# zhaozijie2022/LocoTouch

Measured on AMD Instinct MI355X. Metric: env-steps/sec (whole node), TransportTeacher 4096 envs/GPU, higher is better.
Workload: dtype f32

## Files before the change

locotouch_amd/_abi.py:

```python
from __future__ import annotations

import ctypes
import os
import re

_HERE = os.path.dirname(os.path.abspath(__file__))
REPO = os.path.dirname(_HERE)
LIB_PATH = os.environ.get("LOCOTOUCH_AMD_LIB", os.path.join(_HERE, "_lib", "liblocotouch_env.so"))

_SCALARS = {"int": ctypes.c_int, "int32_t": ctypes.c_int32, "int64_t": ctypes.c_int64, "uint8_t": ctypes.c_uint8,
            "uint32_t": ctypes.c_uint32, "uint64_t": ctypes.c_uint64, "size_t": ctypes.c_size_t, "float": ctypes.c_float,
            "double": ctypes.c_double}
_DECL = re.compile(r"(?:const\s+)?(\w+)\s*((?:\*\s*(?:const\b\s*)?)*)(\w*)\s*((?:\[[^\]]*\]\s*)*)")


def _ctype(decl, structs, opaque, consts, typed, param):
    m = _DECL.fullmatch(decl.strip())
    if not m:
        return None
    base, stars, name, dims = m.groups()
    depth = stars.count("*")
    try:
        dims = [sum(int(t) if t.strip().isdigit() else consts[t.strip()] for t in d.split("+")) for d in re.findall(r"\[([^\]]*)\]", dims)]
    except KeyError:
# ... 42 lines not shown
    protos = {}
    for stmt in filter(None, (x.strip() for x in rest.split(";"))):
        m = re.fullmatch(r"(.*?)\b(\w+)\s*\(([^()]*)\)", stmt, flags=re.S)
        if not m:
            if stmt == "}":
                continue
            raise ImportError(f"cannot parse declaration {stmt!r}")
        ret, name, args = m.groups()
        res = (None, None) if ret.strip() == "void" else _ctype(ret, structs, opaque, consts, typed, param=False)
        args = [] if args.strip() == "void" else [_ctype(a, structs, opaque, consts, typed, param=True) for a in args.split(",")]
        if res is None or None in args:
            raise ImportError(f"cannot type prototype {name}: {' '.join(stmt.split())!r}")
        protos[name] = (res[1], [t for _, t in args])
    return consts, structs, protos


class _CfgMethods(ctypes.Structure):
    def copy(self) -> "LtCfg":
        new = LtCfg()
        ctypes.memmove(ctypes.byref(new), ctypes.byref(self), ctypes.sizeof(self))
        for attr in ("extra_reward_terms", "extra_termination_terms", "extra_observation_terms", "reward_term_params"):
            if hasattr(self, attr):
                v = getattr(self, attr)
                setattr(new, attr, dict(v) if isinstance(v, dict) else list(v))
        return new

    def to_dict(self) -> dict:
        def py(v):
            return [py(x) for x in v] if hasattr(v, "__len__") else v

        return {name: py(getattr(self, name)) for name, *_ in self._fields_ if not name.startswith("_")}


_ENV_VALUE_QUERIES = (
    "lt_abi_version", "lt_cfg_sizeof", "lt_cfg_num_presets", "lt_cfg_preset_id", "lt_cfg_obs_dim", "lt_cfg_tactile_dim", "lt_last_error",
    "lt_wgrad_splits", "lt_wgrad_ws_floats", "lt_elu_backward_bias_ws_floats", "lt_head_wgrad_ws_floats", "lt_adam_clip_step_ws_floats",
    "lt_elu_backward_bias_nblk", "lt_head_wgrad_nblk", "lt_mlp_backward_blocks", "lt_env_kernel_name", "lt_mlp_kernel_name")

HEADERS = (
    ("", "lt_env.h", False, _ENV_VALUE_QUERIES, ("lt_cfg", "lt_view", "lt_mlp_desc", "lt_render_view", "lt_render_desc")),
    ("OBS_NORM", "lt_obs_norm.h", False, (), ()),
    ("STUDENT", "lt_student.h", True, ("lt_student_step_launches",), ("lt_student_desc", "lt_student_params")),
    ("COLLECT", "lt_collect.h", False, (), ()),
    ("LEDGER", "lt_ledger.h", False, (), ()),
    ("CNN_TRAIN", "lt_cnn_train.h", False, ("lt_cnn_launches",), ("lt_cnn_desc", "lt_cnn_params", "lt_cnn_grads")),
    ("BC", "lt_bc.h", False, (), ()),
    ("LSTM", "lt_lstm.h", False, (), ()),
    ("MEMORY", "lt_memory.h", False, (), ("lt_memory_net",)),
    ("MEMORY_SEQ", "lt_memory_seq.h", False, ("lt_memory_seq_backward_units",), ("lt_memory_seq_net", "lt_memory_seq_grad")),
    ("MEMORY_GRU", "lt_memory_gru.h", False, ("lt_memory_gru_seq_backward_units",),
     ("lt_memory_gru_net", "lt_memory_gru_seq_net", "lt_memory_gru_seq_grad")),
    ("POLICY", "lt_policy.h", True, ("lt_policy_step_launches",), ("lt_policy_desc", "lt_policy_memory")),
    ("PPO_OPTS", "lt_ppo_opts.h", False, (), ()),
)


def _bind(table, include_dir):
    bound, seen, env_structs = [], set(), None
    for prefix, fname, uses_env_structs, queries, _ in table:
        path, queries = os.path.join(include_dir, fname), frozenset(queries)
        consts, structs, sigs = parse_header(open(path).read(), structs=env_structs if uses_env_structs else None, bases={"lt_cfg": _CfgMethods})
        if not prefix:
            env_structs = structs
        for name in sorted(queries - set(sigs)):
            raise ImportError(f"include/{fname}: the value query {name} named in _abi.HEADERS is not declared there")
        for name, (restype, _) in sigs.items():
            if name in seen:
                raise ImportError(f"include/{fname}: {name} repeats an entry point of an earlier header")
            if restype is not ctypes.c_int and (prefix or name not in queries):
                raise ImportError(f"include/{fname}: {name} returns no int (a new value query of lt_env.h belongs in _abi.HEADERS)")
        seen.update(sigs)
        bound.append((path, consts, structs, sigs, queries))
    return bound


ALL_SIGNATURES: dict = {}
ALL_VALUE_QUERIES: set = set()
for (_prefix, _, _, _, _published), (_path, _consts, _structs, _sigs, _queries) in zip(HEADERS, _bind(HEADERS, os.path.join(REPO, "include"))):
    _p = _prefix + "_" if _prefix else ""
    globals().update(_consts)
    globals().update({_p + "HEADER": _path, _p + "CONSTS": _consts, _p + "SIGNATURES": _sigs, _p + "VALUE_QUERIES": _queries})
    globals().update({_structs[_c].__name__: _structs[_c] for _c in _published})
    if not _prefix:
        STRUCTS, EXPORTS = _structs, list(_sigs)
    ALL_SIGNATURES.update(_sigs)
    ALL_VALUE_QUERIES |= _queries

_lib = None
_calls: dict = {}


def load() -> ctypes.CDLL:
    global _lib
    if _lib is not None:
        return _lib
    if not os.path.exists(LIB_PATH):
        raise ImportError(f"{LIB_PATH} is missing: run `python -c 'import __graft_entry__ as g; g.build()'` "
                          "(the HIP extension is mandatory, there is no CPU fallback)")
    lib = ctypes.CDLL(LIB_PATH)
    for name, (restype, argtypes) in ALL_SIGNATURES.items():
        fn = getattr(lib, name)
        fn.restype, fn.argtypes = restype, argtypes
        if name not in ALL_VALUE_QUERIES:
            _calls[name] = (fn, [ptr if t is ctypes.c_void_p else _ref if issubclass(t, ctypes._Pointer) and issubclass(t._type_, ctypes.Structure)
                                 else None for t in argtypes])
    if lib.lt_cfg_sizeof() != ctypes.sizeof(LtCfg):
# ... 77 lines not shown
```

locotouch_amd/csrc/lt_ppo.hip:

```cpp
#include <hip/hip_runtime.h>
#include <math.h>
#include <stdint.h>

#include "lt_env.h"
#include "lt_host_check.h"
#include "lt_internal.h"

namespace {

constexpr int MAX_A = 16;
constexpr float kHalfLog2Pi = 0.91893853320467274178f;

__device__ __forceinline__ float lt_sigma_of_log(float log_std) { return (float)exp((double)log_std); }

template <bool LOG, bool NORM>
__global__ __launch_bounds__(256) void lt_ppo_loss_kernel(const float* __restrict__ mu, const float* __restrict__ stdp, const float* __restrict__ value,
                                                          const float* __restrict__ actions, const float* __restrict__ old_logp,
                                                          const float* __restrict__ adv, const float* __restrict__ returns,
                                                          const float* __restrict__ old_values, const float* __restrict__ old_mu,
                                                          const float* __restrict__ old_sigma, const long long* __restrict__ idx,
                                                          long long M, int A, float clip, float vcoef, int clipped_value,
                                                          const float* __restrict__ adv_stats, float* __restrict__ dmu, float* __restrict__ dvalue, float* __restrict__ acc) {
  const long long row = (long long)blockIdx.x * 256 + threadIdx.x;
  const bool ok = row < M;
  const long long src = (ok && idx) ? idx[row] : row;
  __shared__ float sigma_lds[MAX_A];
  if constexpr (LOG) {
    if ((int)threadIdx.x < A) sigma_lds[threadIdx.x] = lt_sigma_of_log(stdp[threadIdx.x]);
    __syncthreads();
  }
  float part[4 + MAX_A];
  float amax_mu = 0.f, amax_v = 0.f;
#pragma unroll
  for (int i = 0; i < 4 + MAX_A; ++i) part[i] = 0.f;
  if (ok) {
    const float inv_m = 1.f / (float)M;
    float logp = 0.f, kl = 0.f;
    float z[MAX_A], isg[MAX_A];
#pragma unroll
    for (int a = 0; a < MAX_A; ++a) {
      if (a < A) {
        const float sg = LOG ? sigma_lds[a] : stdp[a], m = mu[row * A + a], x = actions[src * A + a];
        const float om = old_mu[src * A + a], os = old_sigma[src * A + a];
        isg[a] = 1.f / sg;
        z[a] = (x - m) * isg[a];
        if constexpr (LOG) logp += -0.5f * z[a] * z[a] - stdp[a] - kHalfLog2Pi;
        else logp += -0.5f * z[a] * z[a] - __logf(sg) - kHalfLog2Pi;
        {
#pragma clang fp reciprocal(off)
          kl += logf(sg / os + 1.0e-5f) + (os * os + (om - m) * (om - m)) / (2.f * sg * sg) - 0.5f;
        }
      }
    }
    float advr = adv[src];
    if constexpr (NORM) advr = (advr - adv_stats[0]) * adv_stats[1];
    const float ratio = __expf(logp - old_logp[src]);
    const float s1 = -advr * ratio;
    const float rc = fminf(fmaxf(ratio, 1.f - clip), 1.f + clip);
    const float s2 = -advr * rc;
    const bool inside = ratio >= 1.f - clip && ratio <= 1.f + clip;
    const float dsurr_dratio = (s1 > s2 || inside) ? -advr : 0.f;
    const float dlogp = dsurr_dratio * ratio * inv_m;
#pragma unroll
    for (int a = 0; a < MAX_A; ++a) {
      if (a < A) {
        dmu[row * A + a] = dlogp * z[a] * isg[a];
        amax_mu = fmaxf(amax_mu, fabsf(dlogp * z[a] * isg[a]));
        if constexpr (LOG) part[4 + a] = dlogp * (z[a] * z[a] - 1.f);
        else part[4 + a] = dlogp * (z[a] * z[a] - 1.f) * isg[a];
      }
    }
    const float v = value[row], R = returns[src];
    float vl, dv;
    if (clipped_value) {
      const float ov = old_values[src];
      const float dcl = fminf(fmaxf(v - ov, -clip), clip);
      const float vc = ov + dcl;
      const float l1 = (v - R) * (v - R), l2 = (vc - R) * (vc - R);
      const bool in_v = (v - ov) >= -clip && (v - ov) <= clip;
      vl = fmaxf(l1, l2);
      dv = (l1 > l2 || in_v) ? 2.f * (v - R) : 0.f;
    } else {
      vl = (R - v) * (R - v);
      dv = 2.f * (v - R);
    }
    dvalue[row] = vcoef * dv * inv_m;
    amax_v = fabsf(vcoef * dv * inv_m);
    part[0] = fmaxf(s1, s2);
    part[1] = vl;
    part[2] = kl;
  }
  __shared__ float red[4][4 + MAX_A];
  const int lane = threadIdx.x & 63, wave = threadIdx.x >> 6;
#pragma unroll
  for (int i = 0; i < 4 + MAX_A; ++i) {
    float v = part[i];
#pragma unroll
    for (int off = 32; off > 0; off >>= 1) v += __shfl_xor(v, off, 64);
    if (lane == 0) red[wave][i] = v;
  }
#pragma unroll
  for (int off = 32; off > 0; off >>= 1) {
    amax_mu = fmaxf(amax_mu, __shfl_xor(amax_mu, off, 64));
    amax_v = fmaxf(amax_v, __shfl_xor(amax_v, off, 64));
  }
  __shared__ float redm[4][2];
  if (lane == 0) { redm[wave][0] = amax_mu; redm[wave][1] = amax_v; }
  __syncthreads();
  if (threadIdx.x < 4 + A && threadIdx.x != 3) {
    const int i = threadIdx.x;
    atomicAdd(acc + i, red[0][i] + red[1][i] + red[2][i] + red[3][i]);
  } else if (threadIdx.x >= 64 && threadIdx.x < 66) {
    const int j = threadIdx.x - 64;
    atomicMax((unsigned*)acc + 20 + j, __float_as_uint(fmaxf(fmaxf(redm[0][j], redm[1][j]), fmaxf(redm[2][j], redm[3][j]))));
  }
}

__global__ __launch_bounds__(64) void lt_ppo_finalize_kernel(const float* __restrict__ acc, const float* __restrict__ stdp, int A, float inv_m,
                                                             float vcoef, float ecoef, int std_is_log, float* __restrict__ out) {
  const int a = threadIdx.x;
  float e = 0.f;
  if (a < A && std_is_log) {
    e = 0.5f + kHalfLog2Pi + stdp[a];
    out[8 + a] = acc[4 + a] - ecoef;
  } else if (a < A) {
    const float sg = stdp[a];
    e = 0.5f + kHalfLog2Pi + logf(sg);
    out[8 + a] = acc[4 + a] - ecoef / sg;
  }
  for (int off = 32; off > 0; off >>= 1) e += __shfl_xor(e, off, 64);
  if (a == 0) {
    const float surr = acc[0] * inv_m, vl = acc[1] * inv_m;
    out[0] = surr + vcoef * vl - ecoef * e;
    out[1] = surr; out[2] = vl; out[3] = e; out[4] = acc[2] * inv_m;
  }
}

constexpr int EB_ROWS = 48;

__global__ __launch_bounds__(256) void lt_elu_bwd_bias_kernel(const float* da, const float* __restrict__ a, long long M, int N, float alpha,
                                                              float* dz, float* __restrict__ ws, float* __restrict__ amax) {
  const int n4 = N >> 2, lanes = 256 / n4;
  const int c4 = threadIdx.x % n4, rl = threadIdx.x / n4;
  const long long r0 = (long long)blockIdx.x * EB_ROWS;
  float4 sum = {0.f, 0.f, 0.f, 0.f};
  float mx = 0.f;
  if (rl < lanes) {
    for (int r = rl; r < EB_ROWS; r += lanes) {
      const long long row = r0 + r;
      if (row >= M) break;
      const float4 g = ((const float4*)(da + row * N))[c4], y = ((const float4*)(a + row * N))[c4];
      float4 o;
      o.x = g.x * (y.x > 0.f ? 1.f : y.x + alpha);
      o.y = g.y * (y.y > 0.f ? 1.f : y.y + alpha);
      o.z = g.z * (y.z > 0.f ? 1.f : y.z + alpha);
      o.w = g.w * (y.w > 0.f ? 1.f : y.w + alpha);
      ((float4*)(dz + row * N))[c4] = o;
      sum.x += o.x; sum.y += o.y; sum.z += o.z; sum.w += o.w;
      mx = fmaxf(fmaxf(mx, fmaxf(fabsf(o.x), fabsf(o.y))), fmaxf(fabsf(o.z), fabsf(o.w)));
    }
  }
  __shared__ float4 red[256];
  __shared__ float redm[4];
  red[threadIdx.x] = sum;
  if (amax) {
#pragma unroll
    for (int off = 32; off > 0; off >>= 1) mx = fmaxf(mx, __shfl_xor(mx, off, 64));
    if ((threadIdx.x & 63) == 0) redm[threadIdx.x >> 6] = mx;
  }
  __syncthreads();
  if (amax && threadIdx.x == 0) amax[blockIdx.x] = fmaxf(fmaxf(redm[0], redm[1]), fmaxf(redm[2], redm[3]));
  if (threadIdx.x < n4) {
    float4 t = red[threadIdx.x];
    for (int l = 1; l < lanes; ++l) {
      const float4 u = red[l * n4 + threadIdx.x];
      t.x += u.x; t.y += u.y; t.z += u.z; t.w += u.w;
    }
    ((float4*)(ws + (long long)blockIdx.x * N))[threadIdx.x] = t;
  }
}

constexpr int SUM_MAX_JOBS = 24;
struct SumJobs {
  const float* ws[SUM_MAX_JOBS];
  float* out0[SUM_MAX_JOBS];
  float* out1[SUM_MAX_JOBS];
  long long stride[SUM_MAX_JOBS];
  int nblk[SUM_MAX_JOBS], count[SUM_MAX_JOBS], split[SUM_MAX_JOBS], first[SUM_MAX_JOBS + 1];
// ... 186 lines not shown
    }
  }
  __syncthreads();
  const float coef = s_coef;
  const long long base = (long long)blockIdx.x * AD_PER_BLOCK;
  for (int k = threadIdx.x; k < AD_PER_BLOCK; k += 256) {
    const long long i = base + k;
    if (i >= n) break;
    float gi = g[i] * coef;
    g[i] = gi;
    const float pi = p[i];
    if (wd != 0.f) gi += wd * pi;
    const float mi = m[i] + (1.f - b1) * (gi - m[i]);
    const float vi = b2 * v[i] + (1.f - b2) * gi * gi;
    m[i] = mi;
    v[i] = vi;
    p[i] = pi - step_size * (mi / (sqrtf(vi) / bc2_sqrt + eps));
  }
}

__global__ __launch_bounds__(64) void lt_std_from_log_kernel(const float* __restrict__ log_std, int A, float* __restrict__ stdp) {
  if ((int)threadIdx.x < A) stdp[threadIdx.x] = lt_sigma_of_log(log_std[threadIdx.x]);
}

__device__ __forceinline__ double lt_block_sum_f64(double v, double* red) {
#pragma unroll
  for (int off = 32; off > 0; off >>= 1) v += __shfl_xor(v, off, 64);
  __syncthreads();
  if ((threadIdx.x & 63) == 0) red[threadIdx.x >> 6] = v;
  __syncthreads();
  return (red[0] + red[1]) + (red[2] + red[3]);
}

__global__ __launch_bounds__(256) void lt_adv_stats_kernel(const float* __restrict__ adv, const long long* __restrict__ idx, long long M,
                                                           float* __restrict__ stats) {
#pragma clang fp reciprocal(off)
  __shared__ double red[4];
  const long long base = (long long)blockIdx.x * M;
  double s = 0.0;
  for (long long r = threadIdx.x; r < M; r += 256) s += (double)adv[idx ? idx[base + r] : base + r];
  const double mean = lt_block_sum_f64(s, red) / (double)M;
  double q = 0.0;
  for (long long r = threadIdx.x; r < M; r += 256) {
    const double d = (double)adv[idx ? idx[base + r] : base + r] - mean;
    q += d * d;
  }
  const double var = lt_block_sum_f64(q, red) / (double)(M - 1);
  if (threadIdx.x == 0) {
    stats[2 * blockIdx.x] = (float)mean;
    stats[2 * blockIdx.x + 1] = (float)(1.0 / (sqrt(var) + (double)1.0e-8f));
  }
}

__global__ __launch_bounds__(64) void lt_ppo_lr_rule_kernel(const float* __restrict__ kl_mean, float desired, float lr_min, float lr_max, float factor,
                                                            float* __restrict__ lr, float* __restrict__ stats, const float* __restrict__ scalars,
                                                            float* __restrict__ dstd_out, int A) {
  if (dstd_out && scalars && (int)threadIdx.x < A) dstd_out[threadIdx.x] = scalars[8 + threadIdx.x];
  if (threadIdx.x != 0) return;
  if (kl_mean && desired > 0.f) {
#pragma clang fp reciprocal(off)
    const float kl = *kl_mean;
    float v = *lr;
    if (kl > desired * 2.f) v = fmaxf(lr_min, v / factor);
    else if (kl < desired * 0.5f && kl > 0.f) v = fminf(lr_max, v * factor);
    *lr = v;
  }
  if (stats && scalars) { stats[0] += scalars[2]; stats[1] += scalars[1]; stats[2] += scalars[3]; }
}

}

extern "C" int lt_ppo_lr_rule(const float* kl_mean, float desired_kl, float lr_min, float lr_max, float factor, float* lr, float* stats,
                              const float* scalars, float* dstd_out, int num_actions, void* stream) {
  if (!lr || factor <= 1.f || num_actions < 0 || num_actions > MAX_A) return einval("lt_ppo_lr_rule: invalid argument");
  hipLaunchKernelGGL(lt_ppo_lr_rule_kernel, dim3(1), dim3(64), 0, (hipStream_t)stream, kl_mean, desired_kl, lr_min, lr_max, factor, lr, stats, scalars,
                     dstd_out, num_actions);
  return launch_status();
}

static int elu_backward_bias(const float* da, const float* a, int64_t M, int N, float alpha, float* dz, float* db, float* ws, float* amax, void* stream);
extern "C" int lt_elu_backward_bias(const float* da, const float* a, int64_t M, int N, float alpha, float* dz, float* db, float* ws, void* stream) {
  return elu_backward_bias(da, a, M, N, alpha, dz, db, ws, nullptr, stream);
}
extern "C" int lt_elu_backward_bias2(const float* da, const float* a, int64_t M, int N, float alpha, float* dz, float* db, float* ws, float* amax_blocks,
                                     void* stream) {
  return elu_backward_bias(da, a, M, N, alpha, dz, db, ws, amax_blocks, stream);
}
static int elu_backward_bias(const float* da, const float* a, int64_t M, int N, float alpha, float* dz, float* db, float* ws, float* amax, void* stream) {
  if (!da || !a || !dz || !ws || M < 1 || N < 4 || (N & 3) || N > 1024)
    return einval("lt_elu_backward_bias: invalid argument (N a multiple of 4, 4 <= N <= 1024)");
  const int nblk = (int)((M + EB_ROWS - 1) / EB_ROWS);
  hipLaunchKernelGGL(lt_elu_bwd_bias_kernel, dim3((unsigned)nblk), dim3(256), 0, (hipStream_t)stream, da, a, (long long)M, N, alpha, dz, ws, amax);
  if (db) launch_one_sum(ws, nblk, (long long)N, N, N, db, nullptr, (hipStream_t)stream);
  return launch_status();
}

extern "C" int64_t lt_head_wgrad_ws_floats(int64_t M, int n, int k) { return ((M + HW_ROWS - 1) / HW_ROWS) * ((int64_t)n * k + HW_MAX_N); }

extern "C" int lt_head_wgrad(const float* dy, const float* x, int x_split, int64_t M, int n, int k, float* dw, float* db, float* ws, void* stream) {
  if (!dy || !x || !ws || M < 1 || n < 1 || n > HW_MAX_N || k < 4 || (k & 3) || k > 1024)
    return einval("lt_head_wgrad: invalid argument (1 <= n <= 16, k a multiple of 4, 4 <= k <= 1024)");
  const int nblk = (int)((M + HW_ROWS - 1) / HW_ROWS), k4 = k / 4, lanes = 256 / k4;
  const int nn = n <= 1 ? 1 : (n <= 4 ? 4 : (n <= 8 ? 8 : (n <= 12 ? 12 : 16)));
  const size_t lds = (size_t)lanes * nn * k4 * 16 + (size_t)lanes * nn * 4;
  if (const int e = lt_ensure_dynamic_lds((const void*)lt_head_wgrad_kernel<16>, 72 * 1024)) {
    lt_set_error(hipGetErrorString((hipError_t)e));
    return LT_EHIP;
  }
  if (lds > 72 * 1024) return einval("lt_head_wgrad: n * k too large for one block's LDS partials");
  const dim3 g((unsigned)nblk), b(256);
  hipStream_t st = (hipStream_t)stream;
  switch (nn) {
    case 1: hipLaunchKernelGGL(lt_head_wgrad_kernel<1>, g, b, lds, st, dy, x, x_split, (long long)M, n, k, ws); break;
    case 4: hipLaunchKernelGGL(lt_head_wgrad_kernel<4>, g, b, lds, st, dy, x, x_split, (long long)M, n, k, ws); break;
    case 8: hipLaunchKernelGGL(lt_head_wgrad_kernel<8>, g, b, lds, st, dy, x, x_split, (long long)M, n, k, ws); break;
    case 12: hipLaunchKernelGGL(lt_head_wgrad_kernel<12>, g, b, lds, st, dy, x, x_split, (long long)M, n, k, ws); break;
    default: hipLaunchKernelGGL(lt_head_wgrad_kernel<16>, g, b, lds, st, dy, x, x_split, (long long)M, n, k, ws); break;
  }
  if (dw) launch_one_sum(ws, nblk, (long long)n * k + HW_MAX_N, n * k + n, n * k, dw, db, st);
  return launch_status();
// ... 60 lines not shown

static int ppo_loss(const float* mu, const float* stdp, const float* value, const float* actions, const float* old_logp,
                    const float* adv, const float* returns, const float* old_values, const float* old_mu, const float* old_sigma,
                    const int64_t* idx, int64_t M, int A, float clip, float value_loss_coef, float entropy_coef, int use_clipped_value_loss,
                    int std_is_log, const float* adv_stats, float* dmu, float* dvalue, float* acc, float* out, void* stream) {
  const hipError_t e = hipMemsetAsync(acc, 0, sizeof(float) * (4 + MAX_A + 4), (hipStream_t)stream);
  if (e != hipSuccess) { lt_set_error(hipGetErrorString(e)); return LT_EHIP; }
  const dim3 grid((unsigned)((M + 255) / 256));
#define LT_PPO_LOSS_LAUNCH(LOG, NORM)                                                                                                      \
  hipLaunchKernelGGL((lt_ppo_loss_kernel<LOG, NORM>), grid, dim3(256), 0, (hipStream_t)stream, mu, stdp, value, actions, old_logp, adv, returns, \
                     old_values, old_mu, old_sigma, (const long long*)idx, (long long)M, A, clip, value_loss_coef, use_clipped_value_loss,   \
                     adv_stats, dmu, dvalue, acc)
  if (std_is_log && adv_stats) LT_PPO_LOSS_LAUNCH(true, true);
  else if (std_is_log) LT_PPO_LOSS_LAUNCH(true, false);
  else if (adv_stats) LT_PPO_LOSS_LAUNCH(false, true);
  else LT_PPO_LOSS_LAUNCH(false, false);
#undef LT_PPO_LOSS_LAUNCH
  if (out)
    hipLaunchKernelGGL(lt_ppo_finalize_kernel, dim3(1), dim3(64), 0, (hipStream_t)stream, acc, stdp, A, 1.f / (float)M, value_loss_coef, entropy_coef,
                       std_is_log ? 1 : 0, out);
  return launch_status();
}

extern "C" int lt_ppo_loss(const float* mu, const float* stdp, const float* value, const float* actions, const float* old_logp, const float* adv,
                           const float* returns, const float* old_values, const float* old_mu, const float* old_sigma, const int64_t* idx,
                           int64_t M, int A, float clip, float value_loss_coef, float entropy_coef, int use_clipped_value_loss, float* dmu, float* dvalue,
                           float* acc, float* out, void* stream) {
  if (!mu || !stdp || !value || !actions || !old_logp || !adv || !returns || !old_values || !old_mu || !old_sigma || !dmu || !dvalue || !acc ||
      M < 1 || A < 1 || A > MAX_A)
    return einval("lt_ppo_loss: invalid argument (1 <= num_actions <= 16)");
  return ppo_loss(mu, stdp, value, actions, old_logp, adv, returns, old_values, old_mu, old_sigma, idx, M, A, clip, value_loss_coef,
                  entropy_coef, use_clipped_value_loss, 0, nullptr, dmu, dvalue, acc, out, stream);
}

extern "C" int lt_ppo_loss_opts(const float* mu, const float* stdp, const float* value, const float* actions, const float* old_logp,
                                const float* adv, const float* returns, const float* old_values, const float* old_mu, const float* old_sigma,
                                const int64_t* idx, int64_t M, int A, float clip, float value_loss_coef, float entropy_coef,
                                int use_clipped_value_loss, int std_is_log, const float* adv_stats, float* dmu, float* dvalue, float* acc,
                                float* out, void* stream) {
  const char* fn = "lt_ppo_loss_opts";
  const ptr_check ptrs[] = {{"mu", mu, 4}, {"std", stdp, 4}, {"value", value, 4}, {"actions", actions, 4}, {"old_logp", old_logp, 4}, {"adv", adv, 4},
                            {"returns", returns, 4}, {"old_values", old_values, 4}, {"old_mu", old_mu, 4}, {"old_sigma", old_sigma, 4},
                            {"dmu", dmu, 4}, {"dvalue", dvalue, 4}, {"acc", acc, 4}};
  if (const int rc = check_ptrs(fn, "", ptrs)) return rc;
  if ((uintptr_t)idx % 8 != 0) return refuse(fn, "", "idx", "NULL or 8-byte aligned");
  if ((uintptr_t)adv_stats % 4 != 0) return refuse(fn, "", "adv_stats", "NULL or 4-byte aligned");
  if ((uintptr_t)out % 4 != 0) return refuse(fn, "", "out", "NULL or 4-byte aligned");
  if (M < 1) return refuse(fn, "", "M", ">= 1");
  if (A < 1 || A > MAX_A) return refuse(fn, "", "A", "in [1, 16]");
  return ppo_loss(mu, stdp, value, actions, old_logp, adv, returns, old_values, old_mu, old_sigma, idx, M, A, clip, value_loss_coef, entropy_coef,
                  use_clipped_value_loss, std_is_log, adv_stats, dmu, dvalue, acc, out, stream);
}

extern "C" int lt_std_from_log(const float* log_std, int A, float* stdp, void* stream) {
  const char* fn = "lt_std_from_log";
  const ptr_check ptrs[] = {{"log_std", log_std, 4}, {"std", stdp, 4}};
  if (const int rc = check_ptrs(fn, "", ptrs)) return rc;
  if (A < 1 || A > MAX_A) return refuse(fn, "", "A", "in [1, 16]");
  hipLaunchKernelGGL(lt_std_from_log_kernel, dim3(1), dim3(64), 0, (hipStream_t)stream, log_std, A, stdp);
  return launch_status();
}

extern "C" int lt_adv_stats(const float* adv, const int64_t* idx, int64_t M, int nmb, float* stats, void* stream) {
  const char* fn = "lt_adv_stats";
  const ptr_check ptrs[] = {{"adv", adv, 4}, {"stats", stats, 4}};
  if (const int rc = check_ptrs(fn, "", ptrs)) return rc;
  if ((uintptr_t)idx % 8 != 0) return refuse(fn, "", "idx", "NULL or 8-byte aligned");
  if (M < 2) return refuse(fn, "", "M", ">= 2 (the unbiased std of one element is NaN)");
  if (nmb < 1) return refuse(fn, "", "nmb", ">= 1");
  hipLaunchKernelGGL(lt_adv_stats_kernel, dim3((unsigned)nmb), dim3(256), 0, (hipStream_t)stream, adv, (const long long*)idx, (long long)M, stats);
  return launch_status();
}
```

locotouch_amd/rl/mlp.py:

```python
from __future__ import annotations

import ctypes
import os

import torch
import torch.nn as nn

from .. import _abi

USE_FUSED_BACKWARD = os.environ.get("LT_FUSED_BACKWARD", "1") != "0"
_ACT_IDS = {nn.ELU: "LT_ACT_ELU", nn.ReLU: "LT_ACT_RELU", nn.Tanh: "LT_ACT_TANH", nn.Identity: "LT_ACT_NONE"}


def describe(seq: nn.Sequential):
    linears, acts = [], set()
    mods = list(seq)
    for i, m in enumerate(mods):
        if isinstance(m, nn.Linear):
            if m.bias is None or m.weight.dtype != torch.float32:
                return None
            linears.append(m)
        elif type(m) in _ACT_IDS:
            if type(m) is nn.ELU and (m.alpha != 1.0):
                return None
            if i == 0 or not isinstance(mods[i - 1], nn.Linear) or i == len(mods) - 1:
                return None
            acts.add(type(m))
        else:
            return None
    C = _abi.CONSTS
    if not linears or len(linears) > C["LT_MLP_MAX_LAYERS"] or len(acts) > 1:
        return None
    if len(linears) > 1 and len(mods) != 2 * len(linears) - 1:
        return None
    dims = [linears[0].in_features] + [l.out_features for l in linears]
    if dims[0] > C["LT_MLP_MAX_WIDTH"] or any(d > 512 for d in dims[1:]):
        return None
    if any(a.out_features != b.in_features for a, b in zip(linears[:-1], linears[1:])):
        return None
    desc = _abi.LtMlpDesc()
    desc.num_layers = len(linears)
    for i, d in enumerate(dims):
        desc.dims[i] = d
    desc.activation = C[_ACT_IDS[next(iter(acts))]] if acts else C["LT_ACT_NONE"]
    return desc, linears


class PackedMLP:
    def __init__(self, seq: nn.Sequential):
        got = describe(seq)
        if got is None:
            raise ValueError("network shape not supported by lt_mlp_forward (Linear/activation stack, hidden widths <= 512)")
        self.desc, self.linears = got
        self.lib = _abi.load()
        n = ctypes.c_size_t()
        _abi.call("lt_mlp_packed_floats", self.desc, ctypes.byref(n))
        dev = self.linears[0].weight.device
        self.packed = torch.zeros(n.value, device=dev, dtype=torch.float32)
        self.bpacked = None
        self.in_dtype = torch.float32
        self.out_features = self.linears[-1].out_features
        self.in_features = self.linears[0].in_features
        self.pack()
# ... 351 lines not shown
```

locotouch_amd/rl/ppo.py:

```python
from __future__ import annotations

import torch
import torch.nn as nn

from .. import _abi
from .dist import Dist
from .modules import ActorCritic
from .storage import RolloutStorage


class PPO:
    def __init__(self, actor_critic: ActorCritic, num_learning_epochs=1, num_mini_batches=1, clip_param=0.2, gamma=0.998,
                 lam=0.95, value_loss_coef=1.0, entropy_coef=0.0, learning_rate=1e-3, max_grad_norm=1.0,
                 use_clipped_value_loss=True, schedule="fixed", desired_kl=0.01, device="cpu",
                 normalize_advantage_per_mini_batch=False, dist: Dist | None = None, **unused):
        self.device = device
        self.dist = dist or Dist()
        self.actor_critic = actor_critic.to(device)
        on_gpu = torch.device(device).type == "cuda"
        self.fused_loss = on_gpu and bool(unused.get("fused_loss", True))
        self.packed_forward = on_gpu and bool(unused.get("packed_forward", True))
        self.direct_update = on_gpu and bool(unused.get("direct_update", True))
        self.fused_recurrent_update = bool(unused.get("fused_recurrent_update", False))
        self.fused_gru_memories = bool(unused.get("fused_gru_memories", False))
# ... 98 lines not shown
                try:
                    self._pair = PackedPair(ac.actor, ac.critic)
                except ValueError:
                    self._pair = False
        return self._pair or None

    def _flat_storage(self):
        st = self.storage
        f = lambda t: t.flatten(0, 1)
        small = [f(t).contiguous() for t in (st.actions, st.actions_log_prob, st.advantages, st.returns, st.values, st.mu, st.sigma)]
        return f(st.observations), f(st.privileged_observations), small

    def _fused_update(self):
        from .fused_loss import adv_stats, fused_ppo_loss, std_param

        ac, st = self.actor_critic, self.storage
        obs, cobs, small = self._flat_storage()
        stats = torch.zeros(3, device=obs.device)
        adaptive = self.desired_kl is not None and self.schedule == "adaptive"
        pair = self._packed_pair()
        std_p, std_is_log = std_param(ac)
        if pair is not None and self._flat_adam is not None and self.direct_update and std_p.requires_grad:
            return self._direct_update(pair)
        if pair is not None:
            pair.arm_domain_check()
        perm, mb = st.mini_batch_permutation(self.num_mini_batches)
        mb_stats = adv_stats(small[2], perm, mb, self.num_mini_batches) if self.normalize_advantage_per_mini_batch else None
        for step_i in range(self.num_learning_epochs * self.num_mini_batches):
            i = step_i % self.num_mini_batches
            idx = perm[i * mb:(i + 1) * mb]
            o, co = obs[idx], cobs[idx]
            if o.dtype != torch.float32:
                o, co = o.float(), co.float()
            mu, value = pair(o, co) if pair is not None else (ac.actor(o), ac.critic(co))
            loss, surrogate_loss, value_loss, ent, kl_mean = fused_ppo_loss(
                mu, std_p, value, *small, self.clip_param, self.value_loss_coef, self.entropy_coef,
                self.use_clipped_value_loss, idx=idx, std_is_log=std_is_log, adv_stats=None if mb_stats is None else mb_stats[i])
            kl_handle = self.dist.all_reduce_mean_begin(kl_mean.detach().clone()) if adaptive else None
            self._zero_grad()
            loss.backward()
            if adaptive:
                self._apply_kl(self.dist.all_reduce_mean_end(kl_handle), reduced=True)
            self._optim_step()
            stats = stats + torch.stack((value_loss, surrogate_loss, ent.detach()))
        n = self.num_learning_epochs * self.num_mini_batches
        sv, ss, se = (stats / n).tolist()
        if pair is not None and pair.domain_violated():
            self._warn_mlp_domain()
        st.clear()
        return sv, ss, se, None, None

    def _direct_update(self, pair, split_buckets: bool = True):
        from .fused_loss import adv_stats, std_param

        ac, st, fa = self.actor_critic, self.storage, self._flat_adam
        obs, cobs, small = self._flat_storage()
        small = [t.view(-1) if t.shape[-1] == 1 else t for t in small]
        dev = obs.device
        adaptive = self.desired_kl is not None and self.schedule == "adaptive"
        a_dim = small[0].shape[1]
        state = torch.zeros(4, device=dev)
        state[0] = self.learning_rate
        lr_dev, stats = state[:1], state[1:]
        grad_of = fa.grad_views()
        std_p, std_is_log = std_param(ac)
        std_c = std_p.detach()
        pair.arm_domain_check()
        n_steps = 0
        critic_at = fa.offset_of(next(iter(ac.critic.parameters())))
        two_buckets = split_buckets and 0 < critic_at < self._flat_grad.numel()
        perm, m = st.mini_batch_permutation(self.num_mini_batches)
        perm_o, perm_co = obs[perm], cobs[perm]
        mb_stats = adv_stats(small[2], perm, m, self.num_mini_batches) if self.normalize_advantage_per_mini_batch else None
        if perm_o.dtype != torch.float32:
            perm_o, perm_co = perm_o.float(), perm_co.float()
        split_o = (pair.split_rows(perm_o), pair.split_rows(perm_co)) if pair._fused_backward_possible(perm_o[:m], perm_co[:m]) else None
        for step_i in range(self.num_learning_epochs * self.num_mini_batches):
            i = step_i % self.num_mini_batches
            idx = perm[i * m:(i + 1) * m]
            o, co = perm_o[i * m:(i + 1) * m], perm_co[i * m:(i + 1) * m]
            xs = (split_o[0][i * m:(i + 1) * m], split_o[1][i * m:(i + 1) * m]) if split_o is not None else None
            (mu, value), acts = pair.forward_raw(o, co)
            dmu = torch.empty_like(mu)
            dvalue = torch.empty(m, 1, device=dev, dtype=torch.float32)
            acc = torch.empty(24, device=dev, dtype=torch.float32)
            out = torch.empty(24, device=dev, dtype=torch.float32)
            stream = _abi.stream(dev)
            if std_is_log or mb_stats is not None:
                _abi.call("lt_ppo_loss_opts", mu, std_c, value, *small, idx, m, a_dim, float(self.clip_param), float(self.value_loss_coef),
                          float(self.entropy_coef), int(bool(self.use_clipped_value_loss)), int(std_is_log),
                          None if mb_stats is None else mb_stats[i], dmu, dvalue, acc, out, stream)
            else:
                _abi.call("lt_ppo_loss", mu, std_c, value, *small, idx, m, a_dim, float(self.clip_param), float(self.value_loss_coef),
                          float(self.entropy_coef), int(bool(self.use_clipped_value_loss)), dmu, dvalue, acc, out, stream)
            kl = None
            if adaptive:
                kl = out[4:5]
                if self.dist.world_size > 1:
                    kl = self.dist.all_reduce_mean_(kl.clone())
            _abi.call("lt_ppo_lr_rule", kl, float(self.desired_kl or 0.0), 1e-5, 1e-2, 1.5, lr_dev, stats, out, grad_of[std_p], a_dim, stream)
            if self.dist.world_size > 1 and two_buckets:
                handles = []
                pair.backward_raw(o, co, acts, dmu, dvalue, grad_of, xs, after_first=lambda: handles.append(self.dist.all_reduce_mean_begin(self._flat_grad[:critic_at])),
                                  dy_amax=(acc[20:21], acc[21:22]))
                handles.append(self.dist.all_reduce_mean_begin(self._flat_grad[critic_at:] if handles else self._flat_grad))
                for h in handles:
                    self.dist.all_reduce_mean_end(h)
            else:
                pair.backward_raw(o, co, acts, dmu, dvalue, grad_of, xs, dy_amax=(acc[20:21], acc[21:22]))
                if self.dist.world_size > 1:
                    self.dist.all_reduce_mean_(self._flat_grad)
            fa.step_dev(self.max_grad_norm, lr_dev)
            n_steps += 1
        sat = pair.saturated()
        lr, sv, ss, se, nsat = torch.cat((state, sat if sat is not None else state[:0].new_zeros(1))).tolist()
        if nsat > 0:
            import warnings

            sat.zero_()
            warnings.warn(f"lt_mlp_backward_pair: {int(nsat)} workgroup-layers of the gradient chain reached the f16 image's bound "
                          "(a gradient grew by more than 500x through the layers): those rows were saturated; set LT_FUSED_BACKWARD=0 "
                          "to run the chain as f32 library GEMMs")
        self.learning_rate = lr
        for group in self.optimizer.param_groups:
            group["lr"] = lr
        if pair.domain_violated():
            self._warn_mlp_domain()
        st.clear()
        return sv / n_steps, ss / n_steps, se / n_steps, None, None

    def _warn_mlp_domain(self) -> None:
        import warnings

        self.mlp_domain_violations = getattr(self, "mlp_domain_violations", 0) + 1
        warnings.warn("an observation or hidden activation reached the MLP kernel's saturation bound (|x| >= LT_MLP_INPUT_CLAMP, "
                      "include/lt_env.h): the fused forward computes MLP(clamp(x)) there, unlike the fp32 reference; "
                      "construct PPO(..., packed_forward=False) and FusedRollout(..., use_packed_mlp=False) to run the fp32 GEMM path")

    def _adapt_learning_rate(self, mu, sigma, old_mu, old_sigma) -> None:
        with torch.inference_mode():
            kl = torch.sum(torch.log(sigma / old_sigma + 1.0e-5)
                           + (torch.square(old_sigma) + torch.square(old_mu - mu)) / (2.0 * torch.square(sigma)) - 0.5, dim=-1)
            self._apply_kl(torch.mean(kl))

    def _apply_kl(self, kl_mean, reduced: bool = False) -> None:
        with torch.inference_mode():
            if self.dist.world_size > 1 and not reduced:
                kl_mean = self.dist.all_reduce_mean_(kl_mean.clone())
            kl_mean = float(kl_mean)
        if kl_mean > self.desired_kl * 2.0:
            self.learning_rate = max(1e-5, self.learning_rate / 1.5)
        elif self.desired_kl / 2.0 > kl_mean > 0.0:
            self.learning_rate = min(1e-2, self.learning_rate * 1.5)
        for group in self.optimizer.param_groups:
            group["lr"] = self.learning_rate

    def update(self):
        if self.fused_recurrent_update:
            return self._recurrent_update()
        return self._eager_update()

    def _recurrent_update_unsupported(self) -> str | None:
# ... 165 lines not shown
```

Before: 68.65 million.

## Fuse PPO loss, finalize and LR rule into one last-block kernel

Adds lt_ppo_loss_step, a single kernel that computes the per-row PPO loss and gradients, reduces the partial sums into a persistent workspace, and lets the last block to finish (chosen by an atomic ticket) run the finalize and adaptive-LR rule. The workspace is reset in-kernel by that block. This replaces up to three launches per minibatch (memset/loss, finalize, lr_rule), and the Python loop now reuses preallocated dmu/dvalue/out buffers instead of allocating them each step. It relies on the ticket pattern with relaxed atomics for correctness, and it falls back to the old path for log-std, per-minibatch advantage normalization, or multi-GPU adaptive KL.

```diff
diff --git a/include/lt_ppo_step.h b/include/lt_ppo_step.h
--- /dev/null
+++ b/include/lt_ppo_step.h
@@ -0,0 +1,24 @@
+#ifndef LT_PPO_STEP_H
+#define LT_PPO_STEP_H
+
+#include <stddef.h>
+#include <stdint.h>
+
+#ifdef __cplusplus
+extern "C" {
+#endif
+
+#define LT_PPO_STEP_WS_FLOATS 32
+
+int lt_ppo_loss_step(const float* mu, const float* std, const float* value, const float* actions, const float* old_logp, const float* adv,
+                     const float* returns, const float* old_values, const float* old_mu, const float* old_sigma, const int64_t* idx, int64_t M,
+                     int A, float clip, float value_loss_coef, float entropy_coef, int use_clipped_value_loss, int std_is_log,
+                     const float* adv_stats, float* dmu, float* dvalue, float* ws, float* out, float* dy_amax, int apply_rule, int use_kl,
+                     float desired_kl, float lr_min, float lr_max, float factor, float* lr, float* stats, float* dstd_out, int rows_per_block,
+                     void* stream);
+
+#ifdef __cplusplus
+}
+#endif
+
+#endif
diff --git a/locotouch_amd/_abi.py b/locotouch_amd/_abi.py
--- a/locotouch_amd/_abi.py
+++ b/locotouch_amd/_abi.py
@@ -118,6 +118,7 @@
      ("lt_memory_gru_net", "lt_memory_gru_seq_net", "lt_memory_gru_seq_grad")),
     ("POLICY", "lt_policy.h", True, ("lt_policy_step_launches",), ("lt_policy_desc", "lt_policy_memory")),
     ("PPO_OPTS", "lt_ppo_opts.h", False, (), ()),
+    ("PPO_STEP", "lt_ppo_step.h", False, (), ()),
 )
 
 
diff --git a/locotouch_amd/csrc/lt_ppo.hip b/locotouch_amd/csrc/lt_ppo.hip
--- a/locotouch_amd/csrc/lt_ppo.hip
+++ b/locotouch_amd/csrc/lt_ppo.hip
@@ -5,6 +5,7 @@
 #include "lt_env.h"
 #include "lt_host_check.h"
 #include "lt_internal.h"
+#include "lt_ppo_step.h"
 
 namespace {
 
@@ -13,15 +14,15 @@
 
 __device__ __forceinline__ float lt_sigma_of_log(float log_std) { return (float)exp((double)log_std); }
 
-template <bool LOG, bool NORM>
-__global__ __launch_bounds__(256) void lt_ppo_loss_kernel(const float* __restrict__ mu, const float* __restrict__ stdp, const float* __restrict__ value,
-                                                          const float* __restrict__ actions, const float* __restrict__ old_logp,
-                                                          const float* __restrict__ adv, const float* __restrict__ returns,
-                                                          const float* __restrict__ old_values, const float* __restrict__ old_mu,
-                                                          const float* __restrict__ old_sigma, const long long* __restrict__ idx,
-                                                          long long M, int A, float clip, float vcoef, int clipped_value,
-                                                          const float* __restrict__ adv_stats, float* __restrict__ dmu, float* __restrict__ dvalue, float* __restrict__ acc) {
-  const long long row = (long long)blockIdx.x * 256 + threadIdx.x;
+template <bool LOG, bool NORM, int WAVES, bool DRAIN>
+__device__ __forceinline__ void lt_ppo_loss_rows(const float* __restrict__ mu, const float* __restrict__ stdp, const float* __restrict__ value,
+                                                 const float* __restrict__ actions, const float* __restrict__ old_logp,
+                                                 const float* __restrict__ adv, const float* __restrict__ returns,
+                                                 const float* __restrict__ old_values, const float* __restrict__ old_mu,
+                                                 const float* __restrict__ old_sigma, const long long* __restrict__ idx,
+                                                 long long M, int A, float clip, float vcoef, int clipped_value,
+                                                 const float* __restrict__ adv_stats, float* __restrict__ dmu, float* __restrict__ dvalue, float* acc) {
+  const long long row = (long long)blockIdx.x * (64 * WAVES) + threadIdx.x;
   const bool ok = row < M;
   const long long src = (ok && idx) ? idx[row] : row;
   __shared__ float sigma_lds[MAX_A];
@@ -90,7 +91,7 @@
     part[1] = vl;
     part[2] = kl;
   }
-  __shared__ float red[4][4 + MAX_A];
+  __shared__ float red[WAVES][4 + MAX_A];
   const int lane = threadIdx.x & 63, wave = threadIdx.x >> 6;
 #pragma unroll
   for (int i = 0; i < 4 + MAX_A; ++i) {
@@ -104,36 +105,66 @@
     amax_mu = fmaxf(amax_mu, __shfl_xor(amax_mu, off, 64));
     amax_v = fmaxf(amax_v, __shfl_xor(amax_v, off, 64));
   }
-  __shared__ float redm[4][2];
+  __shared__ float redm[WAVES][2];
   if (lane == 0) { redm[wave][0] = amax_mu; redm[wave][1] = amax_v; }
   __syncthreads();
+  constexpr int MX0 = WAVES > 1 ? 64 : 32;
   if (threadIdx.x < 4 + A && threadIdx.x != 3) {
     const int i = threadIdx.x;
-    atomicAdd(acc + i, red[0][i] + red[1][i] + red[2][i] + red[3][i]);
-  } else if (threadIdx.x >= 64 && threadIdx.x < 66) {
-    const int j = threadIdx.x - 64;
-    atomicMax((unsigned*)acc + 20 + j, __float_as_uint(fmaxf(fmaxf(redm[0][j], redm[1][j]), fmaxf(redm[2][j], redm[3][j]))));
-  }
-}
-
-__global__ __launch_bounds__(64) void lt_ppo_finalize_kernel(const float* __restrict__ acc, const float* __restrict__ stdp, int A, float inv_m,
-                                                             float vcoef, float ecoef, int std_is_log, float* __restrict__ out) {
+    float t = red[0][i];
+#pragma unroll
+    for (int w = 1; w < WAVES; ++w) t += red[w][i];
+    if constexpr (DRAIN) { const float r = atomicAdd(acc + i, t); asm volatile("" ::"v"(r)); }
+    else atomicAdd(acc + i, t);
+  } else if (threadIdx.x >= MX0 && threadIdx.x < MX0 + 2) {
+    const int j = threadIdx.x - MX0;
+    float t = redm[0][j];
+#pragma unroll
+    for (int w = 1; w < WAVES; ++w) t = fmaxf(t, redm[w][j]);
+    if constexpr (DRAIN) { const unsigned r = atomicMax((unsigned*)acc + 20 + j, __float_as_uint(t)); asm volatile("" ::"v"(r)); }
+    else atomicMax((unsigned*)acc + 20 + j, __float_as_uint(t));
+  }
+}
+
+template <bool LOG, bool NORM>
+__global__ __launch_bounds__(256) void lt_ppo_loss_kernel(const float* __restrict__ mu, const float* __restrict__ stdp, const float* __restrict__ value,
+                                                          const float* __restrict__ actions, const float* __restrict__ old_logp,
+                                                          const float* __restrict__ adv, const float* __restrict__ returns,
+                                                          const float* __restrict__ old_values, const float* __restrict__ old_mu,
+                                                          const float* __restrict__ old_sigma, const long long* __restrict__ idx,
+                                                          long long M, int A, float clip, float vcoef, int clipped_value,
+                                                          const float* __restrict__ adv_stats, float* __restrict__ dmu, float* __restrict__ dvalue, float* __restrict__ acc) {
+  lt_ppo_loss_rows<LOG, NORM, 4, false>(mu, stdp, value, actions, old_logp, adv, returns, old_values, old_mu, old_sigma, idx, M, A, clip, vcoef,
+                                        clipped_value, adv_stats, dmu, dvalue, acc);
+}
+
+struct lt_loss_scalars { float surr, vl, e, kl, dstd; };
+
+__device__ __forceinline__ lt_loss_scalars lt_ppo_finalize_wave(float acc_a, float acc0, float acc1, float acc2, const float* __restrict__ stdp, int A,
+                                                                float inv_m, float vcoef, float ecoef, int std_is_log, float* __restrict__ out) {
   const int a = threadIdx.x;
+  lt_loss_scalars r = {0.f, 0.f, 0.f, 0.f, 0.f};
   float e = 0.f;
   if (a < A && std_is_log) {
     e = 0.5f + kHalfLog2Pi + stdp[a];
-    out[8 + a] = acc[4 + a] - ecoef;
+    out[8 + a] = r.dstd = acc_a - ecoef;
   } else if (a < A) {
     const float sg = stdp[a];
     e = 0.5f + kHalfLog2Pi + logf(sg);
-    out[8 + a] = acc[4 + a] - ecoef / sg;
+    out[8 + a] = r.dstd = acc_a - ecoef / sg;
   }
   for (int off = 32; off > 0; off >>= 1) e += __shfl_xor(e, off, 64);
+  r.surr = acc0 * inv_m; r.vl = acc1 * inv_m; r.e = e; r.kl = acc2 * inv_m;
   if (a == 0) {
-    const float surr = acc[0] * inv_m, vl = acc[1] * inv_m;
-    out[0] = surr + vcoef * vl - ecoef * e;
-    out[1] = surr; out[2] = vl; out[3] = e; out[4] = acc[2] * inv_m;
-  }
+    out[0] = r.surr + vcoef * r.vl - ecoef * e;
+    out[1] = r.surr; out[2] = r.vl; out[3] = e; out[4] = r.kl;
+  }
+  return r;
+}
+
+__global__ __launch_bounds__(64) void lt_ppo_finalize_kernel(const float* __restrict__ acc, const float* __restrict__ stdp, int A, float inv_m,
+                                                             float vcoef, float ecoef, int std_is_log, float* __restrict__ out) {
+  lt_ppo_finalize_wave((int)threadIdx.x < A ? acc[4 + threadIdx.x] : 0.f, acc[0], acc[1], acc[2], stdp, A, inv_m, vcoef, ecoef, std_is_log, out);
 }
 
 constexpr int EB_ROWS = 48;
@@ -426,20 +457,63 @@
   }
 }
 
+__device__ __forceinline__ void lt_ppo_lr_rule_lane(bool use_kl, float kl, float desired, float lr_min, float lr_max, float factor, float* __restrict__ lr,
+                                                    float* __restrict__ stats, float vl, float surr, float e) {
+  if (use_kl && desired > 0.f) {
+#pragma clang fp reciprocal(off)
+    float v = *lr;
+    if (kl > desired * 2.f) v = fmaxf(lr_min, v / factor);
+    else if (kl < desired * 0.5f && kl > 0.f) v = fminf(lr_max, v * factor);
+    *lr = v;
+  }
+  if (stats) { stats[0] += vl; stats[1] += surr; stats[2] += e; }
+}
+
 __global__ __launch_bounds__(64) void lt_ppo_lr_rule_kernel(const float* __restrict__ kl_mean, float desired, float lr_min, float lr_max, float factor,
                                                             float* __restrict__ lr, float* __restrict__ stats, const float* __restrict__ scalars,
                                                             float* __restrict__ dstd_out, int A) {
   if (dstd_out && scalars && (int)threadIdx.x < A) dstd_out[threadIdx.x] = scalars[8 + threadIdx.x];
   if (threadIdx.x != 0) return;
-  if (kl_mean && desired > 0.f) {
-#pragma clang fp reciprocal(off)
-    const float kl = *kl_mean;
-    float v = *lr;
-    if (kl > desired * 2.f) v = fmaxf(lr_min, v / factor);
-    else if (kl < desired * 0.5f && kl > 0.f) v = fminf(lr_max, v * factor);
-    *lr = v;
-  }
-  if (stats && scalars) { stats[0] += scalars[2]; stats[1] += scalars[1]; stats[2] += scalars[3]; }
+  const bool st = stats && scalars;
+  lt_ppo_lr_rule_lane(kl_mean != nullptr, kl_mean ? *kl_mean : 0.f, desired, lr_min, lr_max, factor, lr, st ? stats : nullptr, st ? scalars[2] : 0.f,
+                      st ? scalars[1] : 0.f, st ? scalars[3] : 0.f);
+}
+
+struct LossTail {
+  float* ws; float* out; float* dy_amax;
+  float inv_m, ecoef;
+  int std_is_log, apply_rule, use_kl;
+  float desired, lr_min, lr_max, factor;
+  float* lr; float* stats; float* dstd_out;
+};
+
+template <bool LOG, bool NORM, int WAVES>
+__global__ __launch_bounds__(64 * WAVES) void lt_ppo_loss_step_kernel(const float* __restrict__ mu, const float* __restrict__ stdp, const float* __restrict__ value,
+                                                                     const float* __restrict__ actions, const float* __restrict__ old_logp,
+                                                                     const float* __restrict__ adv, const float* __restrict__ returns,
+                                                                     const float* __restrict__ old_values, const float* __restrict__ old_mu,
+                                                                     const float* __restrict__ old_sigma, const long long* __restrict__ idx,
+                                                                     long long M, int A, float clip, float vcoef, int clipped_value,
+                                                                     const float* __restrict__ adv_stats, float* __restrict__ dmu, float* __restrict__ dvalue,
+                                                                     const LossTail T) {
+  lt_ppo_loss_rows<LOG, NORM, WAVES, true>(mu, stdp, value, actions, old_logp, adv, returns, old_values, old_mu, old_sigma, idx, M, A, clip, vcoef,
+                                           clipped_value, adv_stats, dmu, dvalue, T.ws);
+  __shared__ unsigned s_ticket;
+  __syncthreads();
+  if (threadIdx.x == 0) s_ticket = __hip_atomic_fetch_add((unsigned*)T.ws + 24, 1u, __ATOMIC_RELAXED, __HIP_MEMORY_SCOPE_AGENT);
+  __syncthreads();
+  if (s_ticket != gridDim.x - 1 || threadIdx.x >= 64) return;
+  const int lane = threadIdx.x;
+  float v = 0.f;
+  if (lane < 22) v = __hip_atomic_exchange(T.ws + lane, 0.f, __ATOMIC_RELAXED, __HIP_MEMORY_SCOPE_AGENT);
+  else if (lane == 24) __hip_atomic_exchange((unsigned*)T.ws + 24, 0u, __ATOMIC_RELAXED, __HIP_MEMORY_SCOPE_AGENT);
+  if (T.dy_amax && lane >= 20 && lane < 22) T.dy_amax[lane - 20] = v;
+  const float acc_a = __shfl(v, (4 + lane) & 63, 64);
+  const lt_loss_scalars r = lt_ppo_finalize_wave(lane < A ? acc_a : 0.f, __shfl(v, 0, 64), __shfl(v, 1, 64), __shfl(v, 2, 64), stdp, A, T.inv_m, vcoef,
+                                                 T.ecoef, T.std_is_log, T.out);
+  if (!T.apply_rule) return;
+  if (T.dstd_out && lane < A) T.dstd_out[lane] = r.dstd;
+  if (lane == 0) lt_ppo_lr_rule_lane(T.use_kl != 0, r.kl, T.desired, T.lr_min, T.lr_max, T.factor, T.lr, T.stats, r.vl, r.surr, r.e);
 }
 
 }
@@ -606,6 +680,54 @@
                   use_clipped_value_loss, std_is_log, adv_stats, dmu, dvalue, acc, out, stream);
 }
 
+constexpr int LT_PPO_STEP_ROWS = 256;
+
+extern "C" int lt_ppo_loss_step(const float* mu, const float* stdp, const float* value, const float* actions, const float* old_logp, const float* adv,
+                                const float* returns, const float* old_values, const float* old_mu, const float* old_sigma, const int64_t* idx,
+                                int64_t M, int A, float clip, float value_loss_coef, float entropy_coef, int use_clipped_value_loss, int std_is_log,
+                                const float* adv_stats, float* dmu, float* dvalue, float* ws, float* out, float* dy_amax, int apply_rule, int use_kl,
+                                float desired_kl, float lr_min, float lr_max, float factor, float* lr, float* stats, float* dstd_out,
+                                int rows_per_block, void* stream) {
+  const char* fn = "lt_ppo_loss_step";
+  const ptr_check ptrs[] = {{"mu", mu, 4}, {"std", stdp, 4}, {"value", value, 4}, {"actions", actions, 4}, {"old_logp", old_logp, 4}, {"adv", adv, 4},
+                            {"returns", returns, 4}, {"old_values", old_values, 4}, {"old_mu", old_mu, 4}, {"old_sigma", old_sigma, 4},
+                            {"dmu", dmu, 4}, {"dvalue", dvalue, 4}, {"ws", ws, 4}, {"out", out, 4}};
+  if (const int rc = check_ptrs(fn, "", ptrs)) return rc;
+  if ((uintptr_t)idx % 8 != 0) return refuse(fn, "", "idx", "NULL or 8-byte aligned");
+  if ((uintptr_t)adv_stats % 4 != 0) return refuse(fn, "", "adv_stats", "NULL or 4-byte aligned");
+  if ((uintptr_t)dy_amax % 4 != 0) return refuse(fn, "", "dy_amax", "NULL or 4-byte aligned");
+  if (M < 1) return refuse(fn, "", "M", ">= 1");
+  if (A < 1 || A > MAX_A) return refuse(fn, "", "A", "in [1, 16]");
+  if (apply_rule) {
+    if (!lr || (uintptr_t)lr % 4 != 0) return refuse(fn, "", "lr", "non-null and 4-byte aligned (apply_rule != 0)");
+    if (!(factor > 1.f)) return refuse(fn, "", "factor", "> 1 (apply_rule != 0)");
+    if ((uintptr_t)stats % 4 != 0) return refuse(fn, "", "stats", "NULL or 4-byte aligned");
+    if ((uintptr_t)dstd_out % 4 != 0) return refuse(fn, "", "dstd_out", "NULL or 4-byte aligned");
+  }
+  const int rows = rows_per_block ? rows_per_block : LT_PPO_STEP_ROWS;
+  if (rows != 64 && rows != 128 && rows != 256) return refuse(fn, "", "rows_per_block", "0, 64, 128 or 256");
+  const LossTail T = {ws, out, dy_amax, 1.f / (float)M, entropy_coef, std_is_log ? 1 : 0, apply_rule ? 1 : 0, use_kl ? 1 : 0,
+                      desired_kl, lr_min, lr_max, factor, lr, stats, dstd_out};
+  const dim3 grid((unsigned)((M + rows - 1) / rows));
+#define LT_PPO_STEP_LAUNCH(LOG, NORM, WAVES)                                                                                                \
+  hipLaunchKernelGGL((lt_ppo_loss_step_kernel<LOG, NORM, WAVES>), grid, dim3(64 * WAVES), 0, (hipStream_t)stream, mu, stdp, value, actions, old_logp, \
+                     adv, returns, old_values, old_mu, old_sigma, (const long long*)idx, (long long)M, A, clip, value_loss_coef,               \
+                     use_clipped_value_loss, adv_stats, dmu, dvalue, T)
+#define LT_PPO_STEP_FORMS(WAVES)                                        \
+  do {                                                                  \
+    if (std_is_log && adv_stats) LT_PPO_STEP_LAUNCH(true, true, WAVES); \
+    else if (std_is_log) LT_PPO_STEP_LAUNCH(true, false, WAVES);        \
+    else if (adv_stats) LT_PPO_STEP_LAUNCH(false, true, WAVES);         \
+    else LT_PPO_STEP_LAUNCH(false, false, WAVES);                       \
+  } while (0)
+  if (rows == 64) LT_PPO_STEP_FORMS(1);
+  else if (rows == 128) LT_PPO_STEP_FORMS(2);
+  else LT_PPO_STEP_FORMS(4);
+#undef LT_PPO_STEP_FORMS
+#undef LT_PPO_STEP_LAUNCH
+  return launch_status(fn);
+}
+
 extern "C" int lt_std_from_log(const float* log_std, int A, float* stdp, void* stream) {
   const char* fn = "lt_std_from_log";
   const ptr_check ptrs[] = {{"log_std", log_std, 4}, {"std", stdp, 4}};
diff --git a/locotouch_amd/rl/mlp.py b/locotouch_amd/rl/mlp.py
--- a/locotouch_amd/rl/mlp.py
+++ b/locotouch_amd/rl/mlp.py
@@ -9,6 +9,7 @@
 from .. import _abi
 
 USE_FUSED_BACKWARD = os.environ.get("LT_FUSED_BACKWARD", "1") != "0"
+USE_FUSED_PPO_STEP = os.environ.get("LT_FUSED_PPO_STEP", "1") != "0"
 _ACT_IDS = {nn.ELU: "LT_ACT_ELU", nn.ReLU: "LT_ACT_RELU", nn.Tanh: "LT_ACT_TANH", nn.Identity: "LT_ACT_NONE"}
 
 
diff --git a/locotouch_amd/rl/ppo.py b/locotouch_amd/rl/ppo.py
--- a/locotouch_amd/rl/ppo.py
+++ b/locotouch_amd/rl/ppo.py
@@ -174,6 +174,7 @@
 
     def _direct_update(self, pair, split_buckets: bool = True):
         from .fused_loss import adv_stats, std_param
+        from .mlp import USE_FUSED_PPO_STEP as fused_step
 
         ac, st, fa = self.actor_critic, self.storage, self._flat_adam
         obs, cobs, small = self._flat_storage()
@@ -197,39 +198,60 @@
         if perm_o.dtype != torch.float32:
             perm_o, perm_co = perm_o.float(), perm_co.float()
         split_o = (pair.split_rows(perm_o), pair.split_rows(perm_co)) if pair._fused_backward_possible(perm_o[:m], perm_co[:m]) else None
+        fused_loss_step = fused_step and not std_is_log and mb_stats is None
+        if fused_loss_step:
+            if getattr(self, "_step_ws", None) is None or self._step_ws.device != dev:
+                self._step_ws = torch.zeros(_abi.PPO_STEP_CONSTS["LT_PPO_STEP_WS_FLOATS"], device=dev, dtype=torch.float32)
+            else:
+                self._step_ws.zero_()
+            dmu = torch.empty(m, a_dim, device=dev, dtype=torch.float32)
+            dvalue = torch.empty(m, 1, device=dev, dtype=torch.float32)
+            out = torch.empty(24, device=dev, dtype=torch.float32)
+            amax = torch.empty(2, device=dev, dtype=torch.float32)
         for step_i in range(self.num_learning_epochs * self.num_mini_batches):
             i = step_i % self.num_mini_batches
             idx = perm[i * m:(i + 1) * m]
             o, co = perm_o[i * m:(i + 1) * m], perm_co[i * m:(i + 1) * m]
             xs = (split_o[0][i * m:(i + 1) * m], split_o[1][i * m:(i + 1) * m]) if split_o is not None else None
             (mu, value), acts = pair.forward_raw(o, co)
-            dmu = torch.empty_like(mu)
-            dvalue = torch.empty(m, 1, device=dev, dtype=torch.float32)
-            acc = torch.empty(24, device=dev, dtype=torch.float32)
-            out = torch.empty(24, device=dev, dtype=torch.float32)
             stream = _abi.stream(dev)
-            if std_is_log or mb_stats is not None:
-                _abi.call("lt_ppo_loss_opts", mu, std_c, value, *small, idx, m, a_dim, float(self.clip_param), float(self.value_loss_coef),
-                          float(self.entropy_coef), int(bool(self.use_clipped_value_loss)), int(std_is_log),
-                          None if mb_stats is None else mb_stats[i], dmu, dvalue, acc, out, stream)
-            else:
-                _abi.call("lt_ppo_loss", mu, std_c, value, *small, idx, m, a_dim, float(self.clip_param), float(self.value_loss_coef),
-                          float(self.entropy_coef), int(bool(self.use_clipped_value_loss)), dmu, dvalue, acc, out, stream)
-            kl = None
-            if adaptive:
-                kl = out[4:5]
-                if self.dist.world_size > 1:
-                    kl = self.dist.all_reduce_mean_(kl.clone())
-            _abi.call("lt_ppo_lr_rule", kl, float(self.desired_kl or 0.0), 1e-5, 1e-2, 1.5, lr_dev, stats, out, grad_of[std_p], a_dim, stream)
+            if fused_loss_step:
+                rule_here = not (adaptive and self.dist.world_size > 1)
+                _abi.call("lt_ppo_loss_step", mu, std_c, value, *small, idx, m, a_dim, float(self.clip_param), float(self.value_loss_coef),
+                          float(self.entropy_coef), int(bool(self.use_clipped_value_loss)), 0, None, dmu, dvalue, self._step_ws, out, amax,
+                          int(rule_here), int(adaptive),
+                          float(self.desired_kl or 0.0), 1e-5, 1e-2, 1.5, lr_dev, stats, grad_of[std_p], 0, stream)
+                if not rule_here:
+                    kl = self.dist.all_reduce_mean_(out[4:5].clone())
+                    _abi.call("lt_ppo_lr_rule", kl, float(self.desired_kl or 0.0), 1e-5, 1e-2, 1.5, lr_dev, stats, out, grad_of[std_p], a_dim, stream)
+            else:
+                dmu = torch.empty_like(mu)
+                dvalue = torch.empty(m, 1, device=dev, dtype=torch.float32)
+                acc = torch.empty(24, device=dev, dtype=torch.float32)
+                out = torch.empty(24, device=dev, dtype=torch.float32)
+                amax = acc[20:22]
+                if std_is_log or mb_stats is not None:
+                    _abi.call("lt_ppo_loss_opts", mu, std_c, value, *small, idx, m, a_dim, float(self.clip_param), float(self.value_loss_coef),
+                              float(self.entropy_coef), int(bool(self.use_clipped_value_loss)), int(std_is_log),
+                              None if mb_stats is None else mb_stats[i], dmu, dvalue, acc, out, stream)
+                else:
+                    _abi.call("lt_ppo_loss", mu, std_c, value, *small, idx, m, a_dim, float(self.clip_param), float(self.value_loss_coef),
+                              float(self.entropy_coef), int(bool(self.use_clipped_value_loss)), dmu, dvalue, acc, out, stream)
+                kl = None
+                if adaptive:
+                    kl = out[4:5]
+                    if self.dist.world_size > 1:
+                        kl = self.dist.all_reduce_mean_(kl.clone())
+                _abi.call("lt_ppo_lr_rule", kl, float(self.desired_kl or 0.0), 1e-5, 1e-2, 1.5, lr_dev, stats, out, grad_of[std_p], a_dim, stream)
             if self.dist.world_size > 1 and two_buckets:
                 handles = []
                 pair.backward_raw(o, co, acts, dmu, dvalue, grad_of, xs, after_first=lambda: handles.append(self.dist.all_reduce_mean_begin(self._flat_grad[:critic_at])),
-                                  dy_amax=(acc[20:21], acc[21:22]))
+                                  dy_amax=(amax[0:1], amax[1:2]))
                 handles.append(self.dist.all_reduce_mean_begin(self._flat_grad[critic_at:] if handles else self._flat_grad))
                 for h in handles:
                     self.dist.all_reduce_mean_end(h)
             else:
-                pair.backward_raw(o, co, acts, dmu, dvalue, grad_of, xs, dy_amax=(acc[20:21], acc[21:22]))
+                pair.backward_raw(o, co, acts, dmu, dvalue, grad_of, xs, dy_amax=(amax[0:1], amax[1:2]))
                 if self.dist.world_size > 1:
                     self.dist.all_reduce_mean_(self._flat_grad)
             fa.step_dev(self.max_grad_norm, lr_dev)
```

Result: no change. 68.00 million (-1.0%).
